# REEVALUATE/knowledge_enhanced_multimodal_retrieval

Measured on AMD Instinct MI355X. Metric: gallery images+texts encoded/sec (ViT-L/14; synthetic texts per SURVEY 8(d): end-of-text uniform in positions 8..76, mean 43.8 of 77 positions computed -- value_every_text_77_positions is the rate when every text fills the context) and 43k x Q sim+top-10 ms, higher is better.
Workload: dtype bf16; 1 GPU; CLIP ViT-L/14 zero-shot: 43k-gallery encode (1 image + query + target text per item, 224x224 / 77 tokens) + T2I top-10, BASELINE configs[1]; architecture=ViT-L/14, residual_stream=fp24, batch_per_gpu=255, text_group=1501, gallery=43000, parallelism=dp1 (gallery sharded), rccl_ranks=1

## Files before the change

### knowledge_enhanced_multimodal_retrieval_amd/csrc/embed.hip

```cpp
#include "common.h"

namespace kemr {

__global__ __launch_bounds__(256) void im2col_kernel(const float* __restrict__ px, bf16_t* __restrict__ out,
                                                     int image_size, int patch, int grid, int kpad, int kvalid,
                                                     long long total_pairs) {
    const long long gid = (long long)blockIdx.x * 256 + threadIdx.x;
    if (gid >= total_pairs) return;
    const int kp2 = kpad >> 1;
    const long long row = gid / kp2;
    const int k = (int)(gid - row * kp2) * 2;
    const int P = grid * grid;
    const int b = (int)(row / P), pi = (int)(row - (long long)b * P);
    const int py = pi / grid, pxi = pi - py * grid;
    float v[2];
#pragma unroll
    for (int e = 0; e < 2; ++e) {
        const int kk = k + e;
        if (kk < kvalid) {
            const int c = kk / (patch * patch), rem = kk - c * patch * patch;
            const int dy = rem / patch, dx = rem - dy * patch;
            v[e] = px[(((size_t)b * 3 + c) * image_size + (py * patch + dy)) * image_size + pxi * patch + dx];
        } else {
            v[e] = 0.f;
        }
    }
    *(uint32_t*)(out + (size_t)row * kpad + k) = pack_bf16x2(v[0], v[1]);
}

int launch_im2col(const float* pixels, bf16_t* patches, int batch, int image_size, int patch, int kpad, hipStream_t stream) {
    const int grid = image_size / patch;
    const long long pairs = (long long)batch * grid * grid * (kpad / 2);
    if (pairs <= 0) return KEMR_OK;
    const long long blocks = (pairs + 255) / 256;
    if (blocks > 0x7fffffffLL) KEMR_FAIL(KEMR_ERR_INVALID, "im2col: batch too large");
    ProfScope prof(PROF_OTHER, stream);
    hipLaunchKernelGGL(im2col_kernel, dim3((unsigned)blocks), dim3(256), 0, stream, pixels, patches, image_size, patch,
                       grid, kpad, 3 * patch * patch, pairs);
    KEMR_CHECK_LAUNCH("im2col_kernel");
    return KEMR_OK;
}

__global__ __launch_bounds__(256) void cls_rows_kernel(float* __restrict__ x, const float* __restrict__ cls,
                                                       const float* __restrict__ pos, int tokens, int width) {
    const int b = blockIdx.x;
    float* dst = x + (size_t)b * tokens * width;
    for (int i = threadIdx.x; i < width; i += 256) dst[i] = cls[i] + pos[i];
}

int launch_cls_rows(float* x, const float* class_emb, const float* pos, int batch, int tokens, int width, hipStream_t stream) {
    if (batch <= 0) return KEMR_OK;
    ProfScope prof(PROF_OTHER, stream);
    hipLaunchKernelGGL(cls_rows_kernel, dim3(batch), dim3(256), 0, stream, x, class_emb, pos, tokens, width);
    KEMR_CHECK_LAUNCH("cls_rows_kernel");
    return KEMR_OK;
}

__global__ __launch_bounds__(1024) void row_starts_kernel(const int32_t* __restrict__ lens, int batch, int max_len, int rows,
                                                          int* __restrict__ row_start) {
    __shared__ int part[1024];
    const int tid = threadIdx.x, per = (batch + 1023) / 1024;
    const int i0 = tid * per, i1 = i0 + per < batch ? i0 + per : batch;
    int sum = 0;
    for (int i = i0; i < i1; ++i) { const int l = lens[i]; sum += l < 1 ? 1 : (l > max_len ? max_len : l); }
    part[tid] = sum;
    __syncthreads();
    for (int o = 1; o < 1024; o <<= 1) {
        const int v = tid >= o ? part[tid - o] : 0;
        __syncthreads();
// ... 117 lines not shown
    return KEMR_OK;
}

__global__ __launch_bounds__(256) void gather_pooled_kernel(const uint8_t* __restrict__ x, int x_bytes, const uint8_t* __restrict__ h, int h_bytes,
                                                            const int* __restrict__ pool_idx, int width, uint8_t* __restrict__ xc,
                                                            uint8_t* __restrict__ hc) {
    const int b = blockIdx.x;
    const size_t row = (size_t)pool_idx[b];
    const int xb = width * x_bytes, hb = width * h_bytes;
    for (int i = threadIdx.x * 4; i < xb; i += 1024) *(uint32_t*)(xc + (size_t)b * xb + i) = *(const uint32_t*)(x + row * xb + i);
    for (int i = threadIdx.x * 4; i < hb; i += 1024) *(uint32_t*)(hc + (size_t)b * hb + i) = *(const uint32_t*)(h + row * hb + i);
}

int launch_gather_pooled(const void* x, int x_dtype, const void* h, int h_dtype, const int* pool_idx, int batch, int width, void* xc, void* hc,
                         hipStream_t stream) {
    if (batch <= 0) return KEMR_OK;
    if (width % 4) KEMR_FAIL(KEMR_ERR_INVALID, "gather: width %d must be a multiple of 4", width);
    ProfScope prof(PROF_OTHER, stream);
    const int xb = x_dtype == KEMR_BF16 ? 2 : (x_dtype == KEMR_F24 ? 3 : 4), hb = h_dtype == KEMR_FP8 ? 1 : 2;
    hipLaunchKernelGGL(gather_pooled_kernel, dim3(batch), dim3(256), 0, stream, (const uint8_t*)x, xb, (const uint8_t*)h, hb, pool_idx, width,
                       (uint8_t*)xc, (uint8_t*)hc);
    KEMR_CHECK_LAUNCH("gather_pooled_kernel");
    return KEMR_OK;
}

__device__ __forceinline__ float block_sum(float v, float* red) {
    v = wave_sum(v);
    __syncthreads();
    if ((threadIdx.x & 63) == 0) red[threadIdx.x >> 6] = v;
    __syncthreads();
    return (red[0] + red[1]) + (red[2] + red[3]);
}

template <typename XT>
__global__ __launch_bounds__(256) void tail_proj_kernel(const XT* __restrict__ x, const bf16_t* __restrict__ delta,
                                                        const bf16_t* __restrict__ delta2, const int32_t* __restrict__ ids,
                                                        int tokens, int width, const float* __restrict__ gamma,
                                                        const float* __restrict__ beta, const float* __restrict__ proj,
                                                        int d, float* __restrict__ out, const int* __restrict__ row_start,
                                                        float eps, int pool_pos, const float* __restrict__ proj_bias) {
    extern __shared__ __attribute__((aligned(16))) char smem[];
    float* y = (float*)smem;
    float* red = y + width;
    int* pool = (int*)(red + 4);
    const int b = blockIdx.y, tid = threadIdx.x, lane = tid & 63, wid = tid >> 6;

    if (tid < 64) {
        int best_t = pool_pos;
        if (ids) {
            int best_v = INT_MIN;
            best_t = INT_MAX;
            for (int t = tid; t < tokens; t += 64) {
                const int v = ids[(size_t)b * tokens + t];
                if (v > best_v) { best_v = v; best_t = t; }
            }
#pragma unroll
            for (int o = 32; o > 0; o >>= 1) {
                const int ov = __shfl_xor(best_v, o), ot = __shfl_xor(best_t, o);
                if (ov > best_v || (ov == best_v && ot < best_t)) { best_v = ov; best_t = ot; }
            }
        }
        if (tid == 0) *pool = best_t;
    }
    __syncthreads();
    size_t prow = (size_t)b * tokens + *pool;
    if (row_start) {
        const int r0 = row_start[b], len = row_start[b + 1] - r0;
        prow = (size_t)r0 + (*pool < len ? *pool : len - 1);
    }
    const XT* xr = x + prow * width;
    const bf16_t* dr = delta ? delta + prow * width : nullptr;
    const bf16_t* dr2 = delta2 ? delta2 + prow * width : nullptr;

    float s = 0.f;
    for (int i = tid; i < width; i += 256) {
        float v;
        if constexpr (sizeof(XT) == 4) v = xr[i];
        else if constexpr (sizeof(XT) == 3) v = f24_to_f32(((const bf16_t*)xr)[i], ((const uint8_t*)xr)[2 * (size_t)width + i]);
        else v = bf16_to_f32(xr[i]);
        if (dr) v += bf16_to_f32(dr[i]);
        if (dr2) v += bf16_to_f32(dr2[i]);
        y[i] = v;
        s += v;
        if (!proj) out[(size_t)b * width + i] = v;
    }
    if (!proj) return;
    const float mean = block_sum(s, red) / width;
    float q = 0.f;
    for (int i = tid; i < width; i += 256) { const float c = y[i] - mean; q += c * c; }
    const float rstd = 1.0f / sqrtf(block_sum(q, red) / width + eps);
    for (int i = tid; i < width; i += 256) y[i] = (y[i] - mean) * rstd * gamma[i] + beta[i];
    __syncthreads();

    const int j = blockIdx.x * 64 + wid * 16 + (lane & 3) * 4;
    const int g = lane >> 2;
    float4 acc = make_float4(0.f, 0.f, 0.f, 0.f);
    if (j < d) {
#pragma unroll 8
        for (int i = g; i < width; i += 16) {
            const float yi = y[i];
            const float4 p = *(const float4*)(proj + (size_t)i * d + j);
            acc.x = fmaf(yi, p.x, acc.x); acc.y = fmaf(yi, p.y, acc.y);
            acc.z = fmaf(yi, p.z, acc.z); acc.w = fmaf(yi, p.w, acc.w);
        }
    }
#pragma unroll
    for (int o = 4; o < 64; o <<= 1) {
        acc.x += __shfl_xor(acc.x, o); acc.y += __shfl_xor(acc.y, o);
        acc.z += __shfl_xor(acc.z, o); acc.w += __shfl_xor(acc.w, o);
    }
    if (g == 0 && j < d) {
        if (proj_bias) {
            const float4 pb = *(const float4*)(proj_bias + j);
            acc.x += pb.x; acc.y += pb.y; acc.z += pb.z; acc.w += pb.w;
        }
        *(float4*)(out + (size_t)b * d + j) = acc;
    }
}

__global__ __launch_bounds__(256) void l2norm_rows_kernel(float* __restrict__ x, int rows, int d) {
    const int row = blockIdx.x * 4 + (threadIdx.x >> 6), lane = threadIdx.x & 63;
    if (row >= rows) return;
    float* r = x + (size_t)row * d;
    float s = 0.f;
    for (int i = lane; i < d; i += 64) s += r[i] * r[i];
    const float inv = 1.0f / sqrtf(wave_sum(s));
    for (int i = lane; i < d; i += 64) r[i] *= inv;
}

int launch_tail(const void* x, int x_dtype, const bf16_t* delta, const bf16_t* delta2, const int32_t* ids, int batch, int tokens, int width, const float* gamma,
                const float* beta, const float* proj, int d, int normalize, float* out, hipStream_t stream, const int* row_start,
                float eps, int pool_pos, const float* proj_bias) {
    if (batch <= 0) return KEMR_OK;
    if (pool_pos < 0 || pool_pos >= tokens) KEMR_FAIL(KEMR_ERR_INVALID, "tail: pooled position %d outside 0 .. %d", pool_pos, tokens - 1);
    if (d % 4 != 0 || d <= 0) KEMR_FAIL(KEMR_ERR_INVALID, "tail: embed_dim %d must be a positive multiple of 4", d);
    if (batch > 65535) KEMR_FAIL(KEMR_ERR_INVALID, "tail: batch %d > 65535", batch);
    const size_t smem = (size_t)width * 4 + 32;
    ProfScope prof(PROF_OTHER, stream);
    const dim3 grid(proj ? (d + 63) / 64 : 1, batch);
    if (!proj) normalize = 0;
    if (x_dtype == KEMR_BF16)
        hipLaunchKernelGGL(tail_proj_kernel<bf16_t>, grid, dim3(256), smem, stream, (const bf16_t*)x, delta, delta2, ids, tokens, width, gamma, beta, proj, d, out, row_start, eps, pool_pos, proj_bias);
    else if (x_dtype == KEMR_F24)
        hipLaunchKernelGGL(tail_proj_kernel<f24_t>, grid, dim3(256), smem, stream, (const f24_t*)x, delta, delta2, ids, tokens, width, gamma, beta, proj, d, out, row_start, eps, pool_pos, proj_bias);
    else
        hipLaunchKernelGGL(tail_proj_kernel<float>, grid, dim3(256), smem, stream, (const float*)x, delta, delta2, ids, tokens, width, gamma, beta, proj, d, out, row_start, eps, pool_pos, proj_bias);
    KEMR_CHECK_LAUNCH("tail_proj_kernel");
    if (normalize) {
        hipLaunchKernelGGL(l2norm_rows_kernel, dim3((batch + 3) / 4), dim3(256), 0, stream, out, batch, d);
        KEMR_CHECK_LAUNCH("l2norm_rows_kernel");
    }
    return KEMR_OK;
}

template <typename XT>
__global__ __launch_bounds__(256) void stream_cast_kernel(const float* __restrict__ x32, XT* __restrict__ x, int width, long long total4) {
    const long long gid = (long long)blockIdx.x * 256 + threadIdx.x;
    if (gid >= total4) return;
    const int w4 = width >> 2;
    const long long row = gid / w4;
    const int c4 = (int)(gid - row * w4);
    const float4 a = ((const float4*)(x32 + (size_t)row * width))[c4];
    if constexpr (sizeof(XT) == 3) {
        const uint32_t e0 = f32_to_f24_bits(a.x), e1 = f32_to_f24_bits(a.y), e2 = f32_to_f24_bits(a.z), e3 = f32_to_f24_bits(a.w);
        uint8_t* r = (uint8_t*)(x + (size_t)row * width);
        uint2 h;
        h.x = (e0 >> 16) | (e1 & 0xffff0000u);
        h.y = (e2 >> 16) | (e3 & 0xffff0000u);
        ((uint2*)r)[c4] = h;
        ((uint32_t*)(r + 2 * (size_t)width))[c4] = ((e0 >> 8) & 0xff) | (e1 & 0xff00) | ((e2 << 8) & 0xff0000) | ((e3 << 16) & 0xff000000u);
    } else {
        uint2 pk;
        pk.x = pack_bf16x2(a.x, a.y);
        pk.y = pack_bf16x2(a.z, a.w);
        ((uint2*)(x + (size_t)row * width))[c4] = pk;
    }
}

int launch_stream_cast(const float* x32, void* x, int x_dtype, int64_t rows, int width, hipStream_t stream) {
// ... 39 lines not shown
    if (normalize) {
        hipLaunchKernelGGL(l2norm_rows_kernel, dim3((rows + 3) / 4), dim3(256), 0, stream, out, rows, width);
        KEMR_CHECK_LAUNCH("l2norm_rows_kernel");
    }
    return KEMR_OK;
}

template <typename XT>
__device__ __forceinline__ void store_stream4(XT* row, int i4, float4 a, int width) {
    if constexpr (sizeof(XT) == 4) {
        ((float4*)row)[i4] = a;
    } else if constexpr (sizeof(XT) == 3) {
        const uint32_t e0 = f32_to_f24_bits(a.x), e1 = f32_to_f24_bits(a.y), e2 = f32_to_f24_bits(a.z), e3 = f32_to_f24_bits(a.w);
        uint8_t* r = (uint8_t*)row;
        uint2 h;
        h.x = (e0 >> 16) | (e1 & 0xffff0000u);
        h.y = (e2 >> 16) | (e3 & 0xffff0000u);
        ((uint2*)r)[i4] = h;
        ((uint32_t*)(r + 2 * (size_t)width))[i4] = ((e0 >> 8) & 0xff) | (e1 & 0xff00) | ((e2 << 8) & 0xff0000) | ((e3 << 16) & 0xff000000u);
    } else {
        uint2 pk;
        pk.x = pack_bf16x2(a.x, a.y);
        pk.y = pack_bf16x2(a.z, a.w);
        ((uint2*)row)[i4] = pk;
    }
}
template <typename XT>
__device__ __forceinline__ float load_stream1(const XT* row, int i, int width) {
    if constexpr (sizeof(XT) == 4) return row[i];
    else if constexpr (sizeof(XT) == 3) return f24_to_f32(((const bf16_t*)row)[i], ((const uint8_t*)row)[2 * (size_t)width + i]);
    else return bf16_to_f32(row[i]);
}

template <int NV, typename XT>
__global__ __launch_bounds__(256) void bert_embed_kernel(const int32_t* __restrict__ ids, const float* __restrict__ tok, const float* __restrict__ pos,
                                                         const float* __restrict__ gamma, const float* __restrict__ beta, XT* __restrict__ x,
                                                         bf16_t* __restrict__ h, int ctx, int vocab, const int* __restrict__ row_start, int batch,
                                                         int rows, float eps) {
    constexpr int W = NV * 256;
    const int lane = threadIdx.x & 63;
    const int row = blockIdx.x * 4 + (threadIdx.x >> 6);
    if (row >= rows) return;
    int lo = 0, hi = batch - 1;
    while (lo < hi) {
        const int mid = (lo + hi + 1) >> 1;
        if (row_start[mid] <= row) lo = mid; else hi = mid - 1;
    }
    int t = row - row_start[lo];
    t = t < 0 ? 0 : (t < ctx ? t : ctx - 1);
    int id = ids[(size_t)lo * ctx + t];
    id = id < 0 ? 0 : (id >= vocab ? vocab - 1 : id);
    float4 v[NV];
    float s = 0.f;
#pragma unroll
    for (int i = 0; i < NV; ++i) {
        const float4 a = ((const float4*)(tok + (size_t)id * W))[i * 64 + lane];
        const float4 p = ((const float4*)(pos + (size_t)t * W))[i * 64 + lane];
        v[i] = make_float4(a.x + p.x, a.y + p.y, a.z + p.z, a.w + p.w);
        s += (v[i].x + v[i].y) + (v[i].z + v[i].w);
    }
    const float mean = wave_sum(s) * (1.0f / W);
    float q = 0.f;
#pragma unroll
    for (int i = 0; i < NV; ++i) {
        v[i].x -= mean; v[i].y -= mean; v[i].z -= mean; v[i].w -= mean;
        q += (v[i].x * v[i].x + v[i].y * v[i].y) + (v[i].z * v[i].z + v[i].w * v[i].w);
// ... 93 lines not shown
```

### knowledge_enhanced_multimodal_retrieval_amd/csrc/encode.hip

```cpp
#include "model.h"
#include "../../include/kemr_debug.h"

using namespace kemr;

namespace {

int stream_elem_bytes(int x_dtype) { return x_dtype == KEMR_BF16 ? 2 : (x_dtype == KEMR_F24 ? 3 : 4); }

struct Layout { size_t x, h, delta, delta2, big, pool_idx, xc, hc, qc, ac, d1c, d2c, gc, row_start, total; };

Layout ws_layout(int width, int64_t rows, int pooled_items, int x_dtype, int row_starts) {
    const int64_t Mp = round_up(rows, 256), Mc = round_up((int64_t)pooled_items, 256), W = width;
    Layout L{};
    auto take = [&](size_t& at, int64_t bytes) { at = L.total; L.total += (size_t)bytes; };
    take(L.x, round_up(Mp * W * stream_elem_bytes(x_dtype), 256));
    take(L.h, round_up(Mp * W * 2, 256));
    take(L.delta, round_up(Mp * W * 2, 256));
    take(L.delta2, round_up(Mp * W * 2, 256));
    take(L.big, round_up(Mp * W * 8, 256));
    take(L.pool_idx, round_up((int64_t)pooled_items * 4, 256));
    take(L.xc, Mc * W * 4);
    take(L.hc, Mc * W * 2);
    take(L.qc, Mc * W * 2);
    take(L.ac, Mc * W * 2);
// ... 83 lines not shown
    int want_resadd = 0;
    int epi_act = EPI_BIAS_QGELU_BF16;
    float eps = 1e-5f;
    const int* row_start = nullptr;
    int rows = 0;
    int last_pooled = 0;
    const int32_t* ids = nullptr;
    int pool_pos = 0;
};
struct BlockResult {
    bool pending = false;
    bool compact = false;
};

int run_blocks(const TowerW& t, const Workspace& w, int batch, const BlockOpts& o, hipStream_t s, BlockResult& res) {
    const int W = t.width, M = o.row_start ? o.rows : batch * t.tokens;
    const bool fq = o.fp8 & 1, f1 = o.fp8 & 2;
    const int hq = fq ? KEMR_FP8 : KEMR_BF16, h1 = f1 ? KEMR_FP8 : KEMR_BF16;
    bool resadd = o.want_resadd >= (w.x_dtype == KEMR_BF16 ? 1 : 2) && M > 512 && W % 256 == 0 && w.x_dtype != KEMR_F24;
    const int cs = w.x_dtype == KEMR_BF16 ? 2 : 4;
    const int epi_res = w.x_dtype == KEMR_BF16 ? EPI_BIAS_RESADD_BF16 : EPI_BIAS_RESID_F32;
    if (resadd)
        resadd = gemm256u_fits(linear(nullptr, nullptr, nullptr, nullptr, W, M, W, W), 2, cs) &&
                 gemm256u_fits(linear(nullptr, nullptr, nullptr, nullptr, W, M, W, 4 * W), 2, cs);
    res.pending = !resadd && t.layers > 0;
    res.compact = o.last_pooled && !resadd && !f1 && t.layers > 0 && t.tokens <= KEMR_MAX_VISION_TOKENS;
    if (res.compact) KEMR_TRY(launch_pool_index(o.causal ? o.ids : nullptr, o.row_start, batch, t.tokens, w.pool_idx, s, o.pool_pos));
    auto qkv_gemm = [&](const GemmParams& g) { return fq ? launch_gemm256u_fp8(g, EPI_BIAS_BF16, s) : launch_gemm(g, EPI_BIAS_BF16, s); };
    for (int l = 0; l < t.layers; ++l) {
        const LayerW& L = t.layer[l];
        const void* wqkv = fq ? (const void*)L.wqkv8 : (const void*)L.wqkv;
        const size_t wq_bytes = (size_t)W * W * (fq ? 1 : 2);
        if (res.compact && l == t.layers - 1) {
            KEMR_TRY(launch_layernorm(w.x, w.x_dtype, l ? w.delta : nullptr, l ? w.delta2 : nullptr, 1, L.ln1_g, L.ln1_b, w.h, M, W, hq, s, o.eps));
            KEMR_TRY(qkv_gemm(linear(w.h, (const char*)wqkv + wq_bytes, L.bqkv + W, w.big + W, 3 * W, M, 2 * W, W, fq ? L.sqkv + W : nullptr)));
            KEMR_TRY(launch_gather_pooled(w.x, w.x_dtype, w.h, hq, w.pool_idx, batch, W, w.xc, w.hc, s));
            KEMR_TRY(qkv_gemm(linear(w.hc, wqkv, L.bqkv, w.qc, W, batch, W, W, fq ? L.sqkv : nullptr)));
            if (t.head_dim == 80) KEMR_TRY(launch_attention80_pooled(w.qc, w.big, w.ac, batch, t.tokens, W, o.causal, s));
            else KEMR_TRY(launch_attention_pooled(w.qc, w.big, w.ac, w.pool_idx, o.row_start, batch, t.tokens, W, o.causal, s));
            KEMR_TRY(launch_gemm(linear(w.ac, L.wo, L.bo, w.d1c, W, batch, W, W), EPI_BIAS_BF16, s));
            KEMR_TRY(launch_layernorm(w.xc, w.x_dtype, w.d1c, nullptr, 0, L.ln2_g, L.ln2_b, w.hc, batch, W, KEMR_BF16, s, o.eps));
            KEMR_TRY(launch_gemm(linear(w.hc, L.w1, L.b1, w.gc, 4 * W, batch, 4 * W, W), o.epi_act, s));
            KEMR_TRY(launch_gemm(linear(w.gc, L.w2, L.b2, w.d2c, W, batch, W, 4 * W), EPI_BIAS_BF16, s));
            break;
        }
        if (resadd) KEMR_TRY(launch_layernorm(w.x, w.x_dtype, nullptr, nullptr, 0, L.ln1_g, L.ln1_b, w.h, M, W, hq, s, o.eps));
        else KEMR_TRY(launch_layernorm(w.x, w.x_dtype, l ? w.delta : nullptr, l ? w.delta2 : nullptr, 1, L.ln1_g, L.ln1_b, w.h, M, W, hq, s, o.eps));
        KEMR_TRY(qkv_gemm(linear(w.h, wqkv, L.bqkv, w.big, 3 * W, M, 3 * W, W, fq ? L.sqkv : nullptr)));
        if (o.row_start) KEMR_TRY(launch_attention_packed(w.big, w.h, o.row_start, batch, t.tokens, W, s));
        else if (t.head_dim == 80) KEMR_TRY(launch_attention80(w.big, w.h, batch, t.tokens, W, o.causal, s));
        else KEMR_TRY(launch_attention(w.big, w.h, batch, t.tokens, W, o.causal, s));
        KEMR_TRY(launch_gemm(linear(w.h, L.wo, L.bo, resadd ? w.x : (void*)w.delta, W, M, W, W), resadd ? epi_res : EPI_BIAS_BF16, s));
        KEMR_TRY(launch_layernorm(w.x, w.x_dtype, resadd ? nullptr : w.delta, nullptr, 0, L.ln2_g, L.ln2_b, w.h, M, W, h1, s, o.eps));
        if (f1) KEMR_TRY(launch_gemm256u_fp8(linear(w.h, L.w18, L.b1, w.big, 4 * W, M, 4 * W, W, L.s1), o.epi_act, s));
        else KEMR_TRY(launch_gemm(linear(w.h, L.w1, L.b1, w.big, 4 * W, M, 4 * W, W), o.epi_act, s));
        KEMR_TRY(launch_gemm(linear(w.big, L.w2, L.b2, resadd ? w.x : (void*)w.delta2, W, M, W, 4 * W), resadd ? epi_res : EPI_BIAS_BF16, s));
    }
    return KEMR_OK;
}

int check_image_args(const kemr_model* m, const void* pixels_dev, int batch, const void* out_dev, const char* what, bool x3_served) {
    if (!m || !pixels_dev || !out_dev) KEMR_FAIL(KEMR_ERR_INVALID, "%s: null argument", what);
    if (!m->finalized) KEMR_FAIL(KEMR_ERR_STATE, "%s: model not finalized", what);
    if (m->family == 2) KEMR_FAIL(KEMR_ERR_INVALID, "%s: not available for family 2 (BERT): a text-only model has no vision tower", what);
    if (m->x3 && !x3_served) KEMR_FAIL(KEMR_ERR_STATE, "%s: not available for a KEMR_PREC_FP32X3 model", what);
    if (batch < 0) KEMR_FAIL(KEMR_ERR_INVALID, "%s: negative batch", what);
    if (batch > 0 && (int64_t)batch * m->vtokens > (1 << 24)) KEMR_FAIL(KEMR_ERR_INVALID, "%s: batch %d too large", what, batch);
    return KEMR_OK;
}
// ... 299 lines not shown
```

### knowledge_enhanced_multimodal_retrieval_amd/csrc/layernorm.hip

```cpp
#include "common.h"

namespace kemr {

__device__ __forceinline__ float4 load_row4(const float* r, int i, int) { return ((const float4*)r)[i]; }
__device__ __forceinline__ float4 load_row4(const f24_t* r, int i, int W) {
    const uint2 h = ((const uint2*)r)[i];
    const uint32_t l = ((const uint32_t*)((const uint8_t*)r + 2 * (size_t)W))[i];
    return make_float4(f24_to_f32((bf16_t)(h.x & 0xffff), (uint8_t)l), f24_to_f32((bf16_t)(h.x >> 16), (uint8_t)(l >> 8)),
                       f24_to_f32((bf16_t)(h.y & 0xffff), (uint8_t)(l >> 16)), f24_to_f32((bf16_t)(h.y >> 16), (uint8_t)(l >> 24)));
}
typedef unsigned u32x2_nt __attribute__((ext_vector_type(2)));
typedef float f32x4_nt __attribute__((ext_vector_type(4)));
__device__ __forceinline__ float4 load_row4_nt(const float* r, int i, int) {
    const f32x4_nt v = __builtin_nontemporal_load((const f32x4_nt*)r + i);
    return make_float4(v.x, v.y, v.z, v.w);
}
__device__ __forceinline__ float4 load_row4_nt(const f24_t* r, int i, int W) {
    const u32x2_nt h = __builtin_nontemporal_load((const u32x2_nt*)r + i);
    const uint32_t l = __builtin_nontemporal_load((const uint32_t*)((const uint8_t*)r + 2 * (size_t)W) + i);
    return make_float4(f24_to_f32((bf16_t)(h.x & 0xffff), (uint8_t)l), f24_to_f32((bf16_t)(h.x >> 16), (uint8_t)(l >> 8)),
                       f24_to_f32((bf16_t)(h.y & 0xffff), (uint8_t)(l >> 16)), f24_to_f32((bf16_t)(h.y >> 16), (uint8_t)(l >> 24)));
}
__device__ __forceinline__ float4 load_row4_nt(const bf16_t* r, int i, int) {
    const u32x2_nt d = __builtin_nontemporal_load((const u32x2_nt*)r + i);
// ... 47 lines not shown
    int pk = __builtin_amdgcn_cvt_pk_fp8_f32(__builtin_amdgcn_fmed3f(v.x, -lim, lim), __builtin_amdgcn_fmed3f(v.y, -lim, lim), 0, false);
    pk = __builtin_amdgcn_cvt_pk_fp8_f32(__builtin_amdgcn_fmed3f(v.z, -lim, lim), __builtin_amdgcn_fmed3f(v.w, -lim, lim), pk, true);
    ((int*)r)[i] = pk;
}

struct __attribute__((packed)) x3_t { bf16_t v[3]; };
__device__ __forceinline__ void store_row4(x3_t* r, int i, float4 v, int W) {
    uint2 hi, lo;
    split_bf16x2(v.x, v.y, hi.x, lo.x);
    split_bf16x2(v.z, v.w, hi.y, lo.y);
    bf16_t* dst = (bf16_t*)r + 4 * i;
    *(uint2*)dst = hi;
    *(uint2*)(dst + W) = lo;
    *(uint2*)(dst + 2 * W) = hi;
}

template <int NV, typename XT, typename OutT, int MODE, int NTD = 3>
__global__ __launch_bounds__(256) void layernorm_kernel(XT* x, const bf16_t* __restrict__ delta, const bf16_t* __restrict__ delta2,
                                                        const float* __restrict__ gamma, const float* __restrict__ beta,
                                                        OutT* y, int rows, float eps) {
    constexpr int W = NV * 256;
    const int lane = threadIdx.x & 63;
    const int row = blockIdx.x * 4 + (threadIdx.x >> 6);
    if (row >= rows) return;
    XT* xr = x + (size_t)row * W;
    float4 v[NV];
    float s = 0.f;
#pragma unroll
    for (int i = 0; i < NV; ++i) {
        v[i] = NTD >= 2 ? load_row4_nt(xr, i * 64 + lane, W) : load_row4(xr, i * 64 + lane, W);
        if constexpr (MODE != 0) {
            const float4 d = NTD >= 1 ? load_delta4(delta + (size_t)row * W, i * 64 + lane) : load_row4(delta + (size_t)row * W, i * 64 + lane, W);
            v[i].x += d.x; v[i].y += d.y; v[i].z += d.z; v[i].w += d.w;
            if (MODE == 1 && delta2) {
                const float4 e = NTD >= 1 ? load_delta4(delta2 + (size_t)row * W, i * 64 + lane) : load_row4(delta2 + (size_t)row * W, i * 64 + lane, W);
                v[i].x += e.x; v[i].y += e.y; v[i].z += e.z; v[i].w += e.w;
            }
            if constexpr (MODE == 1) {
                if constexpr (NTD >= 3) store_row4_nt(xr, i * 64 + lane, v[i], W);
                else store_row4(xr, i * 64 + lane, v[i], W);
            }
        }
        s += (v[i].x + v[i].y) + (v[i].z + v[i].w);
    }
    const float mean = wave_sum(s) * (1.0f / W);
    float q = 0.f;
#pragma unroll
    for (int i = 0; i < NV; ++i) {
        v[i].x -= mean; v[i].y -= mean; v[i].z -= mean; v[i].w -= mean;
        q += (v[i].x * v[i].x + v[i].y * v[i].y) + (v[i].z * v[i].z + v[i].w * v[i].w);
    }
    const float rstd = 1.0f / sqrtf(wave_sum(q) * (1.0f / W) + eps);
#pragma unroll
    for (int i = 0; i < NV; ++i) {
        const float4 g = ((const float4*)gamma)[i * 64 + lane];
        const float4 b = ((const float4*)beta)[i * 64 + lane];
        float4 o;
        o.x = v[i].x * rstd * g.x + b.x;
        o.y = v[i].y * rstd * g.y + b.y;
        o.z = v[i].z * rstd * g.z + b.z;
        o.w = v[i].w * rstd * g.w + b.w;
        if constexpr (MODE == 3) store_row4_nt(xr, i * 64 + lane, o, W);
        store_row4(y + (size_t)row * W, i * 64 + lane, o, W);
    }
}

// ... 71 lines not shown
        case 768:  return launch_x3_nv<3>(x, gamma, beta, y_panel, rows, stream);
        case 1024: return launch_x3_nv<4>(x, gamma, beta, y_panel, rows, stream);
        case 1280: return launch_x3_nv<5>(x, gamma, beta, y_panel, rows, stream);
    }
    KEMR_FAIL(KEMR_ERR_INVALID, "layernorm_x3: width %d not in {256,512,768,1024,1280}", width);
}

template <typename XT>
static int launch_post_xt(XT* x, const bf16_t* d, const float* g, const float* b, bf16_t* h, int rows, int width, hipStream_t s, float eps) {
    const int blocks = (rows + 3) / 4;
    ProfScope prof(PROF_LAYERNORM, s);
    switch (width) {
        case 256:  hipLaunchKernelGGL((layernorm_kernel<1, XT, bf16_t, 3>), dim3(blocks), dim3(256), 0, s, x, d, (const bf16_t*)nullptr, g, b, h, rows, eps); break;
        case 512:  hipLaunchKernelGGL((layernorm_kernel<2, XT, bf16_t, 3>), dim3(blocks), dim3(256), 0, s, x, d, (const bf16_t*)nullptr, g, b, h, rows, eps); break;
        case 768:  hipLaunchKernelGGL((layernorm_kernel<3, XT, bf16_t, 3>), dim3(blocks), dim3(256), 0, s, x, d, (const bf16_t*)nullptr, g, b, h, rows, eps); break;
        case 1024: hipLaunchKernelGGL((layernorm_kernel<4, XT, bf16_t, 3>), dim3(blocks), dim3(256), 0, s, x, d, (const bf16_t*)nullptr, g, b, h, rows, eps); break;
        case 1280: hipLaunchKernelGGL((layernorm_kernel<5, XT, bf16_t, 3>), dim3(blocks), dim3(256), 0, s, x, d, (const bf16_t*)nullptr, g, b, h, rows, eps); break;
        default: KEMR_FAIL(KEMR_ERR_INVALID, "layernorm_post: width %d not in {256,512,768,1024,1280}", width);
    }
    KEMR_CHECK_LAUNCH("layernorm_kernel (post)");
    return KEMR_OK;
}

int launch_layernorm_post(void* x, int x_dtype, const bf16_t* delta, const float* gamma, const float* beta, bf16_t* h, int rows, int width,
                          hipStream_t stream, float eps) {
    if (rows <= 0) return KEMR_OK;
    if (!delta) KEMR_FAIL(KEMR_ERR_INVALID, "layernorm_post: the post-LN form needs the update it adds");
    if (x_dtype == KEMR_BF16) return launch_post_xt((bf16_t*)x, delta, gamma, beta, h, rows, width, stream, eps);
    if (x_dtype == KEMR_F24) return launch_post_xt((f24_t*)x, delta, gamma, beta, h, rows, width, stream, eps);
    if (x_dtype == KEMR_F32) return launch_post_xt((float*)x, delta, gamma, beta, h, rows, width, stream, eps);
    KEMR_FAIL(KEMR_ERR_INVALID, "layernorm_post: bad row dtype %d", x_dtype);
}

int launch_layernorm(void* x, int x_dtype, const bf16_t* delta, const bf16_t* delta2, int writeback, const float* gamma,
                     const float* beta, void* y, int rows, int width, int out_dtype, hipStream_t stream, float eps) {
    if (rows <= 0) return KEMR_OK;
    if (out_dtype != KEMR_BF16 && out_dtype != KEMR_F32 && out_dtype != KEMR_FP8 && out_dtype != KEMR_F24) KEMR_FAIL(KEMR_ERR_INVALID, "layernorm: bad out dtype %d", out_dtype);
    if (x_dtype != KEMR_BF16 && x_dtype != KEMR_F32 && x_dtype != KEMR_F24) KEMR_FAIL(KEMR_ERR_INVALID, "layernorm: bad row dtype %d", x_dtype);
    if (delta && (out_dtype == KEMR_F32 || out_dtype == KEMR_F24)) KEMR_FAIL(KEMR_ERR_INVALID, "layernorm: the residual forms write bf16 or fp8");
    if (delta2 && !(delta && writeback)) KEMR_FAIL(KEMR_ERR_INVALID, "layernorm: a second delta needs the first one and writeback");
    if (x_dtype == KEMR_BF16) return launch_xt((bf16_t*)x, delta, delta2, writeback, gamma, beta, y, rows, width, out_dtype, stream, eps);
    if (x_dtype == KEMR_F24) return launch_xt((f24_t*)x, delta, delta2, writeback, gamma, beta, y, rows, width, out_dtype, stream, eps);
    return launch_xt((float*)x, delta, delta2, writeback, gamma, beta, y, rows, width, out_dtype, stream, eps);
}

}
```

### knowledge_enhanced_multimodal_retrieval_amd/csrc/model.h

```cpp
#pragma once
#include "common.h"

#include <map>
#include <string>
#include <vector>

namespace kemr {

struct HostTensor {
    std::vector<int64_t> shape;
    std::vector<float> data;
    bool loaded = false;
};

enum TensorTower : int { TOWER_VISION, TOWER_TEXT, TOWER_HEAD };
enum TensorKind : int {
    KIND_F32,
    KIND_MATRIX,
    KIND_QKV_WEIGHT,
    KIND_QKV_BIAS,
    KIND_FC1_WEIGHT,
    KIND_CONV_WEIGHT,
    KIND_LN_QKV,
    KIND_LN_FC1,
// ... 3 lines not shown
};
struct TensorSpec {
    std::string name;
    TensorTower tower;
    int layer;
    TensorKind kind;
    void* bind;
    HostTensor t;
};
struct Placement { size_t off = 0, aux = 0; };
struct PackedWeights {
    size_t bytes = 0;
    std::vector<Placement> at;
    std::vector<char> host;
};

struct LayerW {
    const float *ln1_g, *ln1_b, *ln2_g, *ln2_b, *bqkv, *bo, *b1, *b2;
    const bf16_t *wqkv, *wo, *w1, *w2;
    const uint8_t *wqkv8 = nullptr, *w18 = nullptr;
    const float *sqkv = nullptr, *s1 = nullptr;
};

struct TowerW {
    int width = 0, layers = 0, tokens = 0;
    int head_dim = 64;
    std::vector<LayerW> layer;
};

int fp8_bits(int precision);
int check_finalize(const kemr_model* m, int precision);
void pack_weights(const kemr_model& m, int precision, bool fill, PackedWeights& out);

}

struct kemr_model {
    kemr_cfg cfg;
    std::vector<kemr::TensorSpec> specs;
    std::map<std::string, int> index;
    bool finalized = false;
    char* arena = nullptr;
    size_t arena_bytes = 0;
    int grid = 0, patches = 0, kpad = 0;
    int res_dtype = KEMR_F32;
    int fp8 = 0;
    int resadd = 1;
    int last_pooled = 1;
    int activation = 0;
    int x3 = 0;
    int v_head_dim = 64;
    int stream24 = 1;
    int family = 0;
    int pooling = 0;
    bool any_loaded = false;
    float eps = 1e-5f;
    int vtokens = 0;
    kemr::TowerW vis;
    const kemr::bf16_t* conv_w = nullptr;
    const float *cls = nullptr, *vpos = nullptr, *lnpre_g = nullptr, *lnpre_b = nullptr, *lnpost_g = nullptr,
                *lnpost_b = nullptr, *vproj = nullptr;
    kemr::TowerW txt;
    const float *tok = nullptr, *tpos = nullptr, *lnf_g = nullptr, *lnf_b = nullptr, *tproj = nullptr;
    const float* tproj_b = nullptr;
    const kemr::bf16_t *mh_q = nullptr, *mh_wkv = nullptr, *mh_wo = nullptr, *mh_w1 = nullptr, *mh_w2 = nullptr;
    const float *lne_g = nullptr, *lne_b = nullptr;
    const float *mh_bkv = nullptr, *mh_bo = nullptr, *mh_ln_g = nullptr, *mh_ln_b = nullptr, *mh_b1 = nullptr, *mh_b2 = nullptr;
// ... 2 lines not shown
```

Measured before the change: 18770 items/s.

## Vectorize im2col, batch rows in tail projection, skip residual writeback in last layer

Adds an im2col kernel in which each thread writes eight bf16 outputs with float2 loads and one 16-byte store. The pooled tail projection now handles eight rows per block for widths up to 1280, one row per wave, so each projection weight load is reused across eight rows instead of one. In the last compact layer, a new layernorm mode sums both residual deltas without writing the residual back, and a gather kernel does the same sum only for the pooled rows. Together these cut redundant memory traffic and launches. The cost is more shared memory and registers in the tail kernel.

```diff
diff --git a/knowledge_enhanced_multimodal_retrieval_amd/csrc/embed.hip b/knowledge_enhanced_multimodal_retrieval_amd/csrc/embed.hip
--- a/knowledge_enhanced_multimodal_retrieval_amd/csrc/embed.hip
+++ b/knowledge_enhanced_multimodal_retrieval_amd/csrc/embed.hip
@@ -1,4 +1,6 @@
 #include "common.h"
+
+#include <type_traits>
 
 namespace kemr {
 
@@ -28,6 +30,40 @@
     *(uint32_t*)(out + (size_t)row * kpad + k) = pack_bf16x2(v[0], v[1]);
 }
 
+__global__ __launch_bounds__(256) void im2col8_kernel(const float* __restrict__ px, bf16_t* __restrict__ out,
+                                                      int image_size, int patch, int grid, int kpad, int kvalid,
+                                                      long long total8) {
+    const long long gid = (long long)blockIdx.x * 256 + threadIdx.x;
+    if (gid >= total8) return;
+    const int kp8 = kpad >> 3;
+    const long long row = gid / kp8;
+    const int k0 = (int)(gid - row * kp8) * 8;
+    const int P = grid * grid;
+    const int b = (int)(row / P), pi = (int)(row - (long long)b * P);
+    const int py = pi / grid, pxi = pi - py * grid;
+    const int pp = patch * patch;
+    const int c = k0 / pp, rem = k0 - c * pp;
+    int dy = rem / patch, dx = rem - dy * patch;
+    const size_t plane = (size_t)image_size * image_size;
+    const float* src = px + ((size_t)b * 3 + c) * plane + (size_t)(py * patch + dy) * image_size + pxi * patch + dx;
+    uint32_t w[4];
+#pragma unroll
+    for (int e = 0; e < 4; ++e) {
+        if (k0 + 2 * e < kvalid) {
+            const float2 v = *(const float2*)src;
+            w[e] = pack_bf16x2(v.x, v.y);
+            dx += 2; src += 2;
+            if (dx == patch) {
+                dx = 0; src += image_size - patch;
+                if (++dy == patch) { dy = 0; src += plane - (size_t)patch * image_size; }
+            }
+        } else {
+            w[e] = pack_bf16x2(0.f, 0.f);
+        }
+    }
+    *(uint4*)(out + (size_t)row * kpad + k0) = make_uint4(w[0], w[1], w[2], w[3]);
+}
+
 int launch_im2col(const float* pixels, bf16_t* patches, int batch, int image_size, int patch, int kpad, hipStream_t stream) {
     const int grid = image_size / patch;
     const long long pairs = (long long)batch * grid * grid * (kpad / 2);
@@ -35,6 +71,13 @@
     const long long blocks = (pairs + 255) / 256;
     if (blocks > 0x7fffffffLL) KEMR_FAIL(KEMR_ERR_INVALID, "im2col: batch too large");
     ProfScope prof(PROF_OTHER, stream);
+    if (patch % 2 == 0 && kpad % 8 == 0 && (uintptr_t)pixels % 8 == 0 && (uintptr_t)patches % 16 == 0) {
+        const long long total8 = pairs / 4;
+        hipLaunchKernelGGL(im2col8_kernel, dim3((unsigned)((total8 + 255) / 256)), dim3(256), 0, stream, pixels, patches, image_size, patch,
+                           grid, kpad, 3 * patch * patch, total8);
+        KEMR_CHECK_LAUNCH("im2col_kernel");
+        return KEMR_OK;
+    }
     hipLaunchKernelGGL(im2col_kernel, dim3((unsigned)blocks), dim3(256), 0, stream, pixels, patches, image_size, patch,
                        grid, kpad, 3 * patch * patch, pairs);
     KEMR_CHECK_LAUNCH("im2col_kernel");
@@ -218,25 +261,27 @@
     return (red[0] + red[1]) + (red[2] + red[3]);
 }
 
-template <typename XT>
+constexpr int TAIL_ROWS = 8;
+
+template <typename XT, int R>
 __global__ __launch_bounds__(256) void tail_proj_kernel(const XT* __restrict__ x, const bf16_t* __restrict__ delta,
                                                         const bf16_t* __restrict__ delta2, const int32_t* __restrict__ ids,
                                                         int tokens, int width, const float* __restrict__ gamma,
                                                         const float* __restrict__ beta, const float* __restrict__ proj,
                                                         int d, float* __restrict__ out, const int* __restrict__ row_start,
-                                                        float eps, int pool_pos, const float* __restrict__ proj_bias) {
+                                                        float eps, int pool_pos, const float* __restrict__ proj_bias, int batch) {
     extern __shared__ __attribute__((aligned(16))) char smem[];
-    float* y = (float*)smem;
-    float* red = y + width;
-    int* pool = (int*)(red + 4);
-    const int b = blockIdx.y, tid = threadIdx.x, lane = tid & 63, wid = tid >> 6;
-
-    if (tid < 64) {
+    float* ys = (float*)smem;
+    const int b0 = blockIdx.y * R, tid = threadIdx.x, lane = tid & 63, wid = tid >> 6;
+    const int nr = batch - b0 < R ? batch - b0 : R;
+
+    for (int r = wid; r < nr; r += 4) {
+        const int b = b0 + r;
         int best_t = pool_pos;
         if (ids) {
             int best_v = INT_MIN;
             best_t = INT_MAX;
-            for (int t = tid; t < tokens; t += 64) {
+            for (int t = lane; t < tokens; t += 64) {
                 const int v = ids[(size_t)b * tokens + t];
                 if (v > best_v) { best_v = v; best_t = t; }
             }
@@ -246,61 +291,125 @@
                 if (ov > best_v || (ov == best_v && ot < best_t)) { best_v = ov; best_t = ot; }
             }
         }
-        if (tid == 0) *pool = best_t;
-    }
+        size_t prow = (size_t)b * tokens + best_t;
+        if (row_start) {
+            const int r0 = row_start[b], len = row_start[b + 1] - r0;
+            prow = (size_t)r0 + (best_t < len ? best_t : len - 1);
+        }
+        const XT* xr = x + prow * width;
+        const bf16_t* dr = delta ? delta + prow * width : nullptr;
+        const bf16_t* dr2 = delta2 ? delta2 + prow * width : nullptr;
+        float* y = ys + r * width;
+
+        const bf16_t* dq = dr ? dr : (const bf16_t*)xr;
+        const bf16_t* dq2 = dr2 ? dr2 : (const bf16_t*)xr;
+        float part[4] = {0.f, 0.f, 0.f, 0.f};
+        for (int i0 = lane; i0 < width; i0 += 256) {
+            float v[4], e1[4], e2[4];
+#pragma unroll
+            for (int v4 = 0; v4 < 4; ++v4) {
+                const int i = i0 + v4 * 64, ic = i < width ? i : width - 1;
+                if constexpr (sizeof(XT) == 4) v[v4] = xr[ic];
+                else if constexpr (sizeof(XT) == 3) v[v4] = f24_to_f32(((const bf16_t*)xr)[ic], ((const uint8_t*)xr)[2 * (size_t)width + ic]);
+                else v[v4] = bf16_to_f32(xr[ic]);
+                e1[v4] = bf16_to_f32(dq[ic]);
+                e2[v4] = bf16_to_f32(dq2[ic]);
+            }
+#pragma unroll
+            for (int v4 = 0; v4 < 4; ++v4) {
+                const int i = i0 + v4 * 64;
+                float t = v[v4];
+                t = dr ? t + e1[v4] : t;
+                t = dr2 ? t + e2[v4] : t;
+                if (i < width) {
+                    y[i] = t;
+                    part[v4] += t;
+                    if (!proj) out[(size_t)b * width + i] = t;
+                }
+            }
+        }
+        if (!proj) continue;
+        const float mean = ((wave_sum(part[0]) + wave_sum(part[1])) + (wave_sum(part[2]) + wave_sum(part[3]))) / width;
+        part[0] = part[1] = part[2] = part[3] = 0.f;
+        for (int i0 = lane; i0 < width; i0 += 256) {
+#pragma unroll
+            for (int v4 = 0; v4 < 4; ++v4) {
+                const int i = i0 + v4 * 64;
+                if (i < width) { const float c = y[i] - mean; part[v4] += c * c; }
+            }
+        }
+        const float rstd = 1.0f / sqrtf(((wave_sum(part[0]) + wave_sum(part[1])) + (wave_sum(part[2]) + wave_sum(part[3]))) / width + eps);
+        for (int i0 = lane; i0 < width; i0 += 256) {
+            float ga[4], be[4];
+#pragma unroll
+            for (int v4 = 0; v4 < 4; ++v4) {
+                const int i = i0 + v4 * 64, ic = i < width ? i : width - 1;
+                ga[v4] = gamma[ic]; be[v4] = beta[ic];
+            }
+#pragma unroll
+            for (int v4 = 0; v4 < 4; ++v4) {
+                const int i = i0 + v4 * 64;
+                if (i < width) y[i] = (y[i] - mean) * rstd * ga[v4] + be[v4];
+            }
+        }
+    }
+    if (!proj) return;
     __syncthreads();
-    size_t prow = (size_t)b * tokens + *pool;
-    if (row_start) {
-        const int r0 = row_start[b], len = row_start[b + 1] - r0;
-        prow = (size_t)r0 + (*pool < len ? *pool : len - 1);
-    }
-    const XT* xr = x + prow * width;
-    const bf16_t* dr = delta ? delta + prow * width : nullptr;
-    const bf16_t* dr2 = delta2 ? delta2 + prow * width : nullptr;
-
-    float s = 0.f;
-    for (int i = tid; i < width; i += 256) {
-        float v;
-        if constexpr (sizeof(XT) == 4) v = xr[i];
-        else if constexpr (sizeof(XT) == 3) v = f24_to_f32(((const bf16_t*)xr)[i], ((const uint8_t*)xr)[2 * (size_t)width + i]);
-        else v = bf16_to_f32(xr[i]);
-        if (dr) v += bf16_to_f32(dr[i]);
-        if (dr2) v += bf16_to_f32(dr2[i]);
-        y[i] = v;
-        s += v;
-        if (!proj) out[(size_t)b * width + i] = v;
-    }
-    if (!proj) return;
-    const float mean = block_sum(s, red) / width;
-    float q = 0.f;
-    for (int i = tid; i < width; i += 256) { const float c = y[i] - mean; q += c * c; }
-    const float rstd = 1.0f / sqrtf(block_sum(q, red) / width + eps);
-    for (int i = tid; i < width; i += 256) y[i] = (y[i] - mean) * rstd * gamma[i] + beta[i];
-    __syncthreads();
-
+
+    typedef float f32x4_t __attribute__((ext_vector_type(4)));
     const int j = blockIdx.x * 64 + wid * 16 + (lane & 3) * 4;
     const int g = lane >> 2;
-    float4 acc = make_float4(0.f, 0.f, 0.f, 0.f);
+    float4 acc[R];
+#pragma unroll
+    for (int r = 0; r < R; ++r) acc[r] = make_float4(0.f, 0.f, 0.f, 0.f);
     if (j < d) {
-#pragma unroll 8
-        for (int i = g; i < width; i += 16) {
-            const float yi = y[i];
+        int yoff[R];
+#pragma unroll
+        for (int r = 0; r < R; ++r) yoff[r] = (r < nr ? r : nr - 1) * width;
+        int i = g;
+        for (; i + 16 * 7 < width; i += 16 * 8) {
+            f32x4_t p[8];
+#pragma unroll
+            for (int u = 0; u < 8; ++u) p[u] = *(const f32x4_t*)(proj + (size_t)(i + 16 * u) * d + j);
+            asm volatile("" : "+v"(p[0]), "+v"(p[1]), "+v"(p[2]), "+v"(p[3]), "+v"(p[4]), "+v"(p[5]), "+v"(p[6]), "+v"(p[7]));
+#pragma unroll
+            for (int u = 0; u < 8; ++u) {
+#pragma unroll
+                for (int r = 0; r < R; ++r) {
+                    const float yi = ys[yoff[r] + i + 16 * u];
+                    acc[r].x = fmaf(yi, p[u].x, acc[r].x); acc[r].y = fmaf(yi, p[u].y, acc[r].y);
+                    acc[r].z = fmaf(yi, p[u].z, acc[r].z); acc[r].w = fmaf(yi, p[u].w, acc[r].w);
+                }
+            }
+        }
+        for (; i < width; i += 16) {
             const float4 p = *(const float4*)(proj + (size_t)i * d + j);
-            acc.x = fmaf(yi, p.x, acc.x); acc.y = fmaf(yi, p.y, acc.y);
-            acc.z = fmaf(yi, p.z, acc.z); acc.w = fmaf(yi, p.w, acc.w);
-        }
-    }
-#pragma unroll
-    for (int o = 4; o < 64; o <<= 1) {
-        acc.x += __shfl_xor(acc.x, o); acc.y += __shfl_xor(acc.y, o);
-        acc.z += __shfl_xor(acc.z, o); acc.w += __shfl_xor(acc.w, o);
-    }
-    if (g == 0 && j < d) {
-        if (proj_bias) {
-            const float4 pb = *(const float4*)(proj_bias + j);
-            acc.x += pb.x; acc.y += pb.y; acc.z += pb.z; acc.w += pb.w;
-        }
-        *(float4*)(out + (size_t)b * d + j) = acc;
+#pragma unroll
+            for (int r = 0; r < R; ++r) {
+                const float yi = ys[yoff[r] + i];
+                acc[r].x = fmaf(yi, p.x, acc[r].x); acc[r].y = fmaf(yi, p.y, acc[r].y);
+                acc[r].z = fmaf(yi, p.z, acc[r].z); acc[r].w = fmaf(yi, p.w, acc[r].w);
+            }
+        }
+    }
+    f32x4_t pb = {0.f, 0.f, 0.f, 0.f};
+    if (proj_bias && g == 0 && j < d) pb = *(const f32x4_t*)(proj_bias + j);
+    asm volatile("" : "+v"(pb));
+#pragma unroll
+    for (int r = 0; r < R; ++r) {
+        if (r >= nr) break;
+        float4 a = acc[r];
+#pragma unroll
+        for (int o = 4; o < 64; o <<= 1) {
+            a.x += __shfl_xor(a.x, o); a.y += __shfl_xor(a.y, o);
+            a.z += __shfl_xor(a.z, o); a.w += __shfl_xor(a.w, o);
+        }
+        if (g == 0 && j < d) {
+            if (proj_bias) {
+                a.x += pb.x; a.y += pb.y; a.z += pb.z; a.w += pb.w;
+            }
+            *(float4*)(out + (size_t)(b0 + r) * d + j) = a;
+        }
     }
 }
 
@@ -321,16 +430,22 @@
     if (pool_pos < 0 || pool_pos >= tokens) KEMR_FAIL(KEMR_ERR_INVALID, "tail: pooled position %d outside 0 .. %d", pool_pos, tokens - 1);
     if (d % 4 != 0 || d <= 0) KEMR_FAIL(KEMR_ERR_INVALID, "tail: embed_dim %d must be a positive multiple of 4", d);
     if (batch > 65535) KEMR_FAIL(KEMR_ERR_INVALID, "tail: batch %d > 65535", batch);
-    const size_t smem = (size_t)width * 4 + 32;
-    ProfScope prof(PROF_OTHER, stream);
-    const dim3 grid(proj ? (d + 63) / 64 : 1, batch);
+    ProfScope prof(PROF_OTHER, stream);
     if (!proj) normalize = 0;
-    if (x_dtype == KEMR_BF16)
-        hipLaunchKernelGGL(tail_proj_kernel<bf16_t>, grid, dim3(256), smem, stream, (const bf16_t*)x, delta, delta2, ids, tokens, width, gamma, beta, proj, d, out, row_start, eps, pool_pos, proj_bias);
-    else if (x_dtype == KEMR_F24)
-        hipLaunchKernelGGL(tail_proj_kernel<f24_t>, grid, dim3(256), smem, stream, (const f24_t*)x, delta, delta2, ids, tokens, width, gamma, beta, proj, d, out, row_start, eps, pool_pos, proj_bias);
-    else
-        hipLaunchKernelGGL(tail_proj_kernel<float>, grid, dim3(256), smem, stream, (const float*)x, delta, delta2, ids, tokens, width, gamma, beta, proj, d, out, row_start, eps, pool_pos, proj_bias);
+    auto go = [&](auto xt, auto rows_c) {
+        typedef decltype(xt) XT;
+        constexpr int R = decltype(rows_c)::value;
+        const size_t smem = (size_t)R * width * 4;
+        const dim3 grid(proj ? (d + 63) / 64 : 1, (batch + R - 1) / R);
+        hipLaunchKernelGGL((tail_proj_kernel<XT, R>), grid, dim3(256), smem, stream, (const XT*)x, delta, delta2, ids, tokens, width, gamma, beta, proj, d, out, row_start, eps, pool_pos, proj_bias, batch);
+    };
+    auto by_rows = [&](auto xt) {
+        if (width <= 1280) go(xt, std::integral_constant<int, TAIL_ROWS>());
+        else go(xt, std::integral_constant<int, 1>());
+    };
+    if (x_dtype == KEMR_BF16) by_rows(bf16_t());
+    else if (x_dtype == KEMR_F24) by_rows(f24_t());
+    else by_rows(float());
     KEMR_CHECK_LAUNCH("tail_proj_kernel");
     if (normalize) {
         hipLaunchKernelGGL(l2norm_rows_kernel, dim3((batch + 3) / 4), dim3(256), 0, stream, out, batch, d);
@@ -436,6 +551,43 @@
     else return bf16_to_f32(row[i]);
 }
 
+template <typename XT>
+__global__ __launch_bounds__(256) void gather_pooled_sum_kernel(const XT* __restrict__ x, const bf16_t* __restrict__ d1, const bf16_t* __restrict__ d2,
+                                                                const uint8_t* __restrict__ h, int h_bytes, const int* __restrict__ pool_idx,
+                                                                int width, XT* __restrict__ xc, uint8_t* __restrict__ hc) {
+    const int b = blockIdx.x;
+    const size_t row = (size_t)pool_idx[b];
+    const XT* xr = x + row * width;
+    const bf16_t *r1 = d1 + row * width, *r2 = d2 + row * width;
+    for (int i4 = threadIdx.x; i4 < (width >> 2); i4 += 256) {
+        float v[4];
+#pragma unroll
+        for (int e = 0; e < 4; ++e) {
+            v[e] = load_stream1(xr, 4 * i4 + e, width) + bf16_to_f32(r1[4 * i4 + e]);
+            v[e] += bf16_to_f32(r2[4 * i4 + e]);
+        }
+        store_stream4(xc + (size_t)b * width, i4, make_float4(v[0], v[1], v[2], v[3]), width);
+    }
+    const int hb = width * h_bytes;
+    for (int i = threadIdx.x * 4; i < hb; i += 1024) *(uint32_t*)(hc + (size_t)b * hb + i) = *(const uint32_t*)(h + row * hb + i);
+}
+
+int launch_gather_pooled_sum(const void* x, int x_dtype, const bf16_t* d1, const bf16_t* d2, const void* h, int h_dtype, const int* pool_idx,
+                             int batch, int width, void* xc, void* hc, hipStream_t stream) {
+    if (batch <= 0) return KEMR_OK;
+    if (width % 4) KEMR_FAIL(KEMR_ERR_INVALID, "gather: width %d must be a multiple of 4", width);
+    ProfScope prof(PROF_OTHER, stream);
+    const int hb = h_dtype == KEMR_FP8 ? 1 : 2;
+    if (x_dtype == KEMR_BF16)
+        hipLaunchKernelGGL(gather_pooled_sum_kernel<bf16_t>, dim3(batch), dim3(256), 0, stream, (const bf16_t*)x, d1, d2, (const uint8_t*)h, hb, pool_idx, width, (bf16_t*)xc, (uint8_t*)hc);
+    else if (x_dtype == KEMR_F24)
+        hipLaunchKernelGGL(gather_pooled_sum_kernel<f24_t>, dim3(batch), dim3(256), 0, stream, (const f24_t*)x, d1, d2, (const uint8_t*)h, hb, pool_idx, width, (f24_t*)xc, (uint8_t*)hc);
+    else
+        hipLaunchKernelGGL(gather_pooled_sum_kernel<float>, dim3(batch), dim3(256), 0, stream, (const float*)x, d1, d2, (const uint8_t*)h, hb, pool_idx, width, (float*)xc, (uint8_t*)hc);
+    KEMR_CHECK_LAUNCH("gather_pooled_kernel");
+    return KEMR_OK;
+}
+
 template <int NV, typename XT>
 __global__ __launch_bounds__(256) void bert_embed_kernel(const int32_t* __restrict__ ids, const float* __restrict__ tok, const float* __restrict__ pos,
                                                          const float* __restrict__ gamma, const float* __restrict__ beta, XT* __restrict__ x,
diff --git a/knowledge_enhanced_multimodal_retrieval_amd/csrc/encode.hip b/knowledge_enhanced_multimodal_retrieval_amd/csrc/encode.hip
--- a/knowledge_enhanced_multimodal_retrieval_amd/csrc/encode.hip
+++ b/knowledge_enhanced_multimodal_retrieval_amd/csrc/encode.hip
@@ -139,9 +139,11 @@
         const void* wqkv = fq ? (const void*)L.wqkv8 : (const void*)L.wqkv;
         const size_t wq_bytes = (size_t)W * W * (fq ? 1 : 2);
         if (res.compact && l == t.layers - 1) {
-            KEMR_TRY(launch_layernorm(w.x, w.x_dtype, l ? w.delta : nullptr, l ? w.delta2 : nullptr, 1, L.ln1_g, L.ln1_b, w.h, M, W, hq, s, o.eps));
+            if (l) KEMR_TRY(launch_layernorm_sum2(w.x, w.x_dtype, w.delta, w.delta2, L.ln1_g, L.ln1_b, w.h, M, W, hq, s, o.eps));
+            else KEMR_TRY(launch_layernorm(w.x, w.x_dtype, nullptr, nullptr, 1, L.ln1_g, L.ln1_b, w.h, M, W, hq, s, o.eps));
             KEMR_TRY(qkv_gemm(linear(w.h, (const char*)wqkv + wq_bytes, L.bqkv + W, w.big + W, 3 * W, M, 2 * W, W, fq ? L.sqkv + W : nullptr)));
-            KEMR_TRY(launch_gather_pooled(w.x, w.x_dtype, w.h, hq, w.pool_idx, batch, W, w.xc, w.hc, s));
+            if (l) KEMR_TRY(launch_gather_pooled_sum(w.x, w.x_dtype, w.delta, w.delta2, w.h, hq, w.pool_idx, batch, W, w.xc, w.hc, s));
+            else KEMR_TRY(launch_gather_pooled(w.x, w.x_dtype, w.h, hq, w.pool_idx, batch, W, w.xc, w.hc, s));
             KEMR_TRY(qkv_gemm(linear(w.hc, wqkv, L.bqkv, w.qc, W, batch, W, W, fq ? L.sqkv : nullptr)));
             if (t.head_dim == 80) KEMR_TRY(launch_attention80_pooled(w.qc, w.big, w.ac, batch, t.tokens, W, o.causal, s));
             else KEMR_TRY(launch_attention_pooled(w.qc, w.big, w.ac, w.pool_idx, o.row_start, batch, t.tokens, W, o.causal, s));
diff --git a/knowledge_enhanced_multimodal_retrieval_amd/csrc/layernorm.hip b/knowledge_enhanced_multimodal_retrieval_amd/csrc/layernorm.hip
--- a/knowledge_enhanced_multimodal_retrieval_amd/csrc/layernorm.hip
+++ b/knowledge_enhanced_multimodal_retrieval_amd/csrc/layernorm.hip
@@ -103,6 +103,10 @@
         if constexpr (MODE != 0) {
             const float4 d = NTD >= 1 ? load_delta4(delta + (size_t)row * W, i * 64 + lane) : load_row4(delta + (size_t)row * W, i * 64 + lane, W);
             v[i].x += d.x; v[i].y += d.y; v[i].z += d.z; v[i].w += d.w;
+            if constexpr (MODE == 4) {
+                const float4 e = load_delta4(delta2 + (size_t)row * W, i * 64 + lane);
+                v[i].x += e.x; v[i].y += e.y; v[i].z += e.z; v[i].w += e.w;
+            }
             if (MODE == 1 && delta2) {
                 const float4 e = NTD >= 1 ? load_delta4(delta2 + (size_t)row * W, i * 64 + lane) : load_row4(delta2 + (size_t)row * W, i * 64 + lane, W);
                 v[i].x += e.x; v[i].y += e.y; v[i].z += e.z; v[i].w += e.w;
@@ -240,6 +244,38 @@
     KEMR_FAIL(KEMR_ERR_INVALID, "layernorm_post: bad row dtype %d", x_dtype);
 }
 
+template <typename XT, typename OutT>
+static int launch_sum2_xt(const XT* x, const bf16_t* d1, const bf16_t* d2, const float* g, const float* b, OutT* y, int rows, int width,
+                          hipStream_t s, float eps) {
+    const int blocks = (rows + 3) / 4;
+    ProfScope prof(PROF_LAYERNORM, s);
+    switch (width) {
+        case 256:  hipLaunchKernelGGL((layernorm_kernel<1, XT, OutT, 4>), dim3(blocks), dim3(256), 0, s, (XT*)x, d1, d2, g, b, y, rows, eps); break;
+        case 512:  hipLaunchKernelGGL((layernorm_kernel<2, XT, OutT, 4>), dim3(blocks), dim3(256), 0, s, (XT*)x, d1, d2, g, b, y, rows, eps); break;
+        case 768:  hipLaunchKernelGGL((layernorm_kernel<3, XT, OutT, 4>), dim3(blocks), dim3(256), 0, s, (XT*)x, d1, d2, g, b, y, rows, eps); break;
+        case 1024: hipLaunchKernelGGL((layernorm_kernel<4, XT, OutT, 4>), dim3(blocks), dim3(256), 0, s, (XT*)x, d1, d2, g, b, y, rows, eps); break;
+        case 1280: hipLaunchKernelGGL((layernorm_kernel<5, XT, OutT, 4>), dim3(blocks), dim3(256), 0, s, (XT*)x, d1, d2, g, b, y, rows, eps); break;
+        default: KEMR_FAIL(KEMR_ERR_INVALID, "layernorm: width %d not in {256,512,768,1024,1280}", width);
+    }
+    KEMR_CHECK_LAUNCH("layernorm_kernel");
+    return KEMR_OK;
+}
+
+int launch_layernorm_sum2(const void* x, int x_dtype, const bf16_t* delta, const bf16_t* delta2, const float* gamma, const float* beta, void* y,
+                          int rows, int width, int out_dtype, hipStream_t stream, float eps) {
+    if (rows <= 0) return KEMR_OK;
+    if (out_dtype != KEMR_BF16 && out_dtype != KEMR_FP8) KEMR_FAIL(KEMR_ERR_INVALID, "layernorm: the residual forms write bf16 or fp8");
+    if (x_dtype != KEMR_BF16 && x_dtype != KEMR_F32 && x_dtype != KEMR_F24) KEMR_FAIL(KEMR_ERR_INVALID, "layernorm: bad row dtype %d", x_dtype);
+    if (!delta || !delta2) KEMR_FAIL(KEMR_ERR_INVALID, "layernorm: the two-delta form without write-back needs both deltas");
+    const bool f8 = out_dtype == KEMR_FP8;
+    if (x_dtype == KEMR_BF16) return f8 ? launch_sum2_xt((const bf16_t*)x, delta, delta2, gamma, beta, (fp8_t*)y, rows, width, stream, eps)
+                                        : launch_sum2_xt((const bf16_t*)x, delta, delta2, gamma, beta, (bf16_t*)y, rows, width, stream, eps);
+    if (x_dtype == KEMR_F24) return f8 ? launch_sum2_xt((const f24_t*)x, delta, delta2, gamma, beta, (fp8_t*)y, rows, width, stream, eps)
+                                       : launch_sum2_xt((const f24_t*)x, delta, delta2, gamma, beta, (bf16_t*)y, rows, width, stream, eps);
+    return f8 ? launch_sum2_xt((const float*)x, delta, delta2, gamma, beta, (fp8_t*)y, rows, width, stream, eps)
+              : launch_sum2_xt((const float*)x, delta, delta2, gamma, beta, (bf16_t*)y, rows, width, stream, eps);
+}
+
 int launch_layernorm(void* x, int x_dtype, const bf16_t* delta, const bf16_t* delta2, int writeback, const float* gamma,
                      const float* beta, void* y, int rows, int width, int out_dtype, hipStream_t stream, float eps) {
     if (rows <= 0) return KEMR_OK;
diff --git a/knowledge_enhanced_multimodal_retrieval_amd/csrc/model.h b/knowledge_enhanced_multimodal_retrieval_amd/csrc/model.h
--- a/knowledge_enhanced_multimodal_retrieval_amd/csrc/model.h
+++ b/knowledge_enhanced_multimodal_retrieval_amd/csrc/model.h
@@ -59,6 +59,11 @@
 int check_finalize(const kemr_model* m, int precision);
 void pack_weights(const kemr_model& m, int precision, bool fill, PackedWeights& out);
 
+int launch_layernorm_sum2(const void* x, int x_dtype, const bf16_t* delta, const bf16_t* delta2, const float* gamma, const float* beta, void* y,
+                          int rows, int width, int out_dtype , hipStream_t stream, float eps = 1e-5f);
+int launch_gather_pooled_sum(const void* x, int x_dtype, const bf16_t* d1, const bf16_t* d2, const void* h, int h_dtype, const int* pool_idx,
+                             int batch, int width, void* xc, void* hc, hipStream_t stream);
+
 }
 
 struct kemr_model {
```

Measured after the change: 18880 items/s (median of 6 runs). No clear change (+0.5%).
